# eBay/Sequence-Semantic-Embedding

Measured on AMD Instinct MI355X. Metric: encoded seqs/sec (+ query x target cosine-scores/sec, top-1 vs ref), higher is better.
Workload: dtype f32; 1 GPU; configs[1]: classification stand-in, dual-encoder LSTM H=S=256 E=50 T=32 V=32000; encode 16384 source seqs/GPU/step + cosine top-10 vs 571-target index; batch_per_gpu=16384, seq_len=32, targets=571, parallelism=dp1, weights=random-init (reference initialisers, seed 0)

## Files before the change

### sequence-semantic-embedding_amd/csrc/score_topk.hip

```cpp
#include <cstdlib>

#include "sse_kernels.h"
#include "score_exact.h"

#define SC_THREADS 512
#define SC_KC 16
#ifndef SC_PRIO_K
#define SC_PRIO_K 1
#define SC_PRIO_E 0
#endif

#ifdef SSE_SCORE_CLOCK
#include <cstdio>
__device__ long long g_score_clk[8 * 8];
#define SC_CLK_DECL long long ck_[8] = {0, 0, 0, 0, 0, 0, 0, 0}, ck_t = clock64();
#define SC_CLK(i)                   \
  {                                 \
    const long long n_ = clock64(); \
    ck_[i] += n_ - ck_t;            \
    ck_t = n_;                      \
  }
#else
#define SC_CLK_DECL
#define SC_CLK(i)
// ... 983 lines not shown
      col[row] = (row < a.N) ? acc[r] : NEG_INF;
    }
  }
  SC_CLK(1)
  __syncthreads();
  SC_CLK(2)
  if (NT * 32 <= 640) {
    si_select4<10>(a, sc, NP, NT, qt, w * 8, lane SI_CLK_ARGS);
    SC_CLK(3)
    si_select4<10>(a, sc, NP, NT, qt, w * 8 + 4, lane SI_CLK_ARGS);
    SC_CLK(4)
#ifdef SSE_SCORE_CLOCK
    if (blockIdx.x == gridDim.x / 2 && lane == 0)
      for (int i = 0; i < 8; ++i) g_score_clk[w * 8 + i] = ck_[i];
#endif
  } else {
    si_select4<16>(a, sc, NP, NT, qt, w * 8, lane SI_CLK_ARGS);
    si_select4<16>(a, sc, NP, NT, qt, w * 8 + 4, lane SI_CLK_ARGS);
  }
}
template <int KB>
__global__ __launch_bounds__(256) void score_small_index_x3_kernel(SmallIndexArgs a) {
  extern __shared__ __attribute__((aligned(16))) float si_sc[];
  const int tid = threadIdx.x, lane = tid & 63, w = __builtin_amdgcn_readfirstlane(tid >> 6);
  const int NT = a.NT, NP = NT * 32 + 1;
  const int qt = blockIdx.x;
  float *sc = si_sc;
  SC_CLK_DECL
  sse_u32x4 bh[KB], bl[KB];
  {
    const int row = qt * 32 + (lane & 31), kb0 = (lane >> 5) * 8;
    const float *src = a.q_rows + (size_t)(row < a.Q ? row : 0) * a.S + kb0;
    const bool vec = (a.S & 3) == 0 && (reinterpret_cast<uintptr_t>(a.q_rows) & 15) == 0 && KB * 16 <= a.S;
#pragma unroll
    for (int kb = 0; kb < KB; ++kb) {
      float v[8] = {0, 0, 0, 0, 0, 0, 0, 0};
      if (vec) {
        const f32x4 v0 = *reinterpret_cast<const f32x4 *>(src + kb * 16), v1 = *reinterpret_cast<const f32x4 *>(src + kb * 16 + 4);
#pragma unroll
        for (int e = 0; e < 4; ++e) {
          v[e] = v0[e];
          v[4 + e] = v1[e];
        }
      } else {
#pragma unroll
        for (int e = 0; e < 8; ++e)
          if (kb * 16 + kb0 + e < a.S) v[e] = src[kb * 16 + e];
      }
      if (row >= a.Q) {
#pragma unroll
        for (int e = 0; e < 8; ++e) v[e] = 0.0f;
      }
      sse_split8(v, bh[kb], bl[kb]);
    }
  }
  SC_CLK(0)
  {
    constexpr int D = KB < 4 ? KB : 4;
    static_assert(KB % D == 0, "the ring index must be static");
    const sse_u32x4 *img = reinterpret_cast<const sse_u32x4 *>(a.idx_x3) + lane;
    const sse_u32x4 *ap = img + (size_t)(w < NT ? w : 0) * KB * 128;
    sse_u32x4 ah[D], al[D];
#pragma unroll
    for (int d = 0; d < D; ++d) {
      ah[d] = ap[d * 128];
      al[d] = ap[d * 128 + 64];
    }
    for (int t = w; t < NT; t += 4) {
      const sse_u32x4 *apn = img + (size_t)(t + 4 < NT ? t + 4 : t) * KB * 128;
      f32x16 acc = {0, 0, 0, 0, 0, 0, 0, 0, 0, 0, 0, 0, 0, 0, 0, 0};
#pragma unroll
      for (int kb = 0; kb < KB; ++kb) {
        __builtin_amdgcn_sched_barrier(0);
        const bf16x8_t xh = __builtin_bit_cast(bf16x8_t, ah[kb % D]), xl = __builtin_bit_cast(bf16x8_t, al[kb % D]);
        const bf16x8_t yh = __builtin_bit_cast(bf16x8_t, bh[kb]), yl = __builtin_bit_cast(bf16x8_t, bl[kb]);
        acc = __builtin_amdgcn_mfma_f32_32x32x16_bf16(xh, yh, acc, 0, 0, 0);
        acc = __builtin_amdgcn_mfma_f32_32x32x16_bf16(xh, yl, acc, 0, 0, 0);
        acc = __builtin_amdgcn_mfma_f32_32x32x16_bf16(xl, yh, acc, 0, 0, 0);
        __builtin_amdgcn_sched_barrier(0);
        const sse_u32x4 *nx = (kb + D < KB) ? ap + (kb + D) * 128 : apn + (kb + D - KB) * 128;
        ah[kb % D] = nx[0];
        al[kb % D] = nx[64];
      }
      const int rb = t * 32 + 4 * (lane >> 5);
      float *col = sc + (lane & 31) * NP;
#pragma unroll
      for (int r = 0; r < 16; ++r) {
        const int row = rb + (r & 3) + 8 * (r >> 2);
        col[row] = (row < a.N) ? acc[r] : NEG_INF;
      }
      ap = apn;
    }
  }
  SC_CLK(1)
  __syncthreads();
  SC_CLK(2)
  if (NT * 32 <= 640) {
    si_select4<10>(a, sc, NP, NT, qt, w * 8, lane SI_CLK_ARGS);
    SC_CLK(3)
    si_select4<10>(a, sc, NP, NT, qt, w * 8 + 4, lane SI_CLK_ARGS);
    SC_CLK(4)
#ifdef SSE_SCORE_CLOCK
    if (blockIdx.x == gridDim.x / 2 && lane == 0)
      for (int i = 0; i < 8; ++i) g_score_clk[w * 8 + i] = ck_[i];
#endif
  } else {
    si_select4<16>(a, sc, NP, NT, qt, w * 8, lane SI_CLK_ARGS);
    si_select4<16>(a, sc, NP, NT, qt, w * 8 + 4, lane SI_CLK_ARGS);
  }
}
bool score_small_index_applies(int Q, int KG, int64_t NT) {
  return Q >= 1024 && (KG == 32 || KG == 8 || KG == 7) && NT * 32 <= 1024 && (size_t)32 * (NT * 32 + 1) * sizeof(float) <= (size_t)144 * 1024;
}
hipError_t launch_score_small_index(const SmallIndexArgs &a, hipStream_t stream) {
  if (!score_small_index_applies(a.Q, a.KG, a.NT)) return hipErrorInvalidValue;
  const size_t lds = (size_t)32 * (a.NT * 32 + 1) * sizeof(float);
  const dim3 grid((a.Q + 31) / 32), block(256);
  auto go = [&](auto kernel) -> hipError_t {
    hipError_t e = hipFuncSetAttribute(reinterpret_cast<const void *>(kernel), hipFuncAttributeMaxDynamicSharedMemorySize, (int)lds);
    if (e != hipSuccess) return e;
    hipLaunchKernelGGL(kernel, grid, block, lds, stream, a);
    return hipGetLastError();
  };
  if (a.idx_x3 && a.KG != 32) return go(score_small_index_x3_kernel<4>);
  if (a.KG == 8) return go(score_small_index_kernel<8>);
  if (a.KG == 7) return go(score_small_index_kernel<7>);
  const hipError_t e32 = a.idx_x3 ? go(score_small_index_x3_kernel<16>) : go(score_small_index_kernel<32>);
  if (e32 != hipSuccess) return e32;
#ifdef SSE_SCORE_CLOCK
  if (a.Q >= 8192) {
    static int n = 0;
    if (n++ % 8 == 3) {
      long long v[64];
      (void)hipStreamSynchronize(stream);
      (void)hipMemcpyFromSymbol(v, HIP_SYMBOL(g_score_clk), sizeof v);
      for (int w = 0; w < 4; w += 3)
        fprintf(stderr, "[small index clock Q=%d NT=%d] wave %d cycles: query fragments %lld | scores (MFMA + LDS stores) %lld | barrier %lld | selection: loads + bounds %lld | bisection %lld | winners + rank + stores %lld (both batches)\n",
                a.Q, a.NT, w, v[w * 8 + 0], v[w * 8 + 1], v[w * 8 + 2], v[w * 8 + 5], v[w * 8 + 6], v[w * 8 + 3] + v[w * 8 + 4]);
    }
  }
#endif
  return hipGetLastError();
}

hipError_t launch_score_topk(const ScoreArgs &a_in, hipStream_t stream) {
  ScoreArgs a = a_in;
#ifdef SSE_SCORE_MEASURE
  {
    static const int dbg = getenv("SSE_SCORE_DBG") ? atoi(getenv("SSE_SCORE_DBG")) : 0;
// ... 11 lines not shown
    if (a.NQ == 2) return launch_score_variant<2, false, true>(a, stream);
    if (a.NQ == 4) return launch_score_variant<4, false, true>(a, stream);
    return hipErrorInvalidValue;
  }
  if (!a.part_bnd) return hipErrorInvalidValue;
  if (a.BF) {
    if (a.NQ == 1) return launch_score_variant<1, true, false>(a, stream);
    if (a.NQ == 2) return launch_score_variant<2, true, false>(a, stream);
    if (a.NQ == 4) return launch_score_variant<4, true, false>(a, stream);
    return hipErrorInvalidValue;
  }
  if (a.NQ == 1) return launch_score_variant<1, false, false>(a, stream);
  if (a.NQ == 2) return launch_score_variant<2, false, false>(a, stream);
  if (a.NQ == 4) return launch_score_variant<4, false, false>(a, stream);
  return hipErrorInvalidValue;
}


template <int NB>
__device__ __forceinline__ int packed_value_of_lane(int lane) {
  int v = 0;
#pragma unroll
  for (int cnt = NB, bit = 5; cnt > 1; cnt >>= 1, --bit) v = v * 2 + ((lane >> bit) & 1);
  return v;
}
template <int NB>
__device__ __forceinline__ int packed_lane_of_value(int v) {
  int lane = 0;
#pragma unroll
  for (int cnt = NB, bit = 5; cnt > 1; cnt >>= 1, --bit) lane |= ((v / (cnt / 2)) & 1) << bit;
  return lane;
}
template <int NB>
__device__ __forceinline__ double wave_exact_dot_packed(const float *qrow, const float *idxp, const double *idx64, const int64_t (&n)[NB],
                                                        int S, int KG, int lane, const float *idx_rm = nullptr) {
  static_assert(NB == 2 || NB == 4 || NB == 8, "power of two");
  double acc[NB];
#pragma unroll
  for (int b = 0; b < NB; ++b) acc[b] = 0.0;
  if (idx64) {
    for (int d = lane; d < S; d += 64) {
      double rv[NB];
#pragma unroll
      for (int b = 0; b < NB; ++b) rv[b] = idx64[(size_t)n[b] * S + d];
#pragma unroll
      for (int b = 0; b < NB; ++b) acc[b] += (double)qrow[d] * rv[b];
    }
  } else {
    for (int j = lane; j < KG * 2; j += 64) {
      const int kg = j >> 1, half = j & 1;
      f32x4 v[NB];
#pragma unroll
      for (int b = 0; b < NB; ++b)
        v[b] = idx_rm ? *reinterpret_cast<const f32x4 *>(idx_rm + (size_t)n[b] * S + j * 4)
                      : *reinterpret_cast<const f32x4 *>(idxp + (size_t)(n[b] >> 5) * KG * 256 + kg * 256 + (half * 32 + (int)(n[b] & 31)) * 4);
      const int d0 = kg * 8 + half * 4;
#pragma unroll
      for (int e = 0; e < 4; ++e)
        if (d0 + e < S) {
#pragma unroll
          for (int b = 0; b < NB; ++b) acc[b] += (double)qrow[d0 + e] * (double)v[b][e];
        }
    }
  }
  int m = 32;
#pragma unroll
  for (int cnt = NB; cnt > 1; cnt >>= 1, m >>= 1) {
    const bool up = (lane & m) != 0;
#pragma unroll
    for (int i = 0; i < cnt / 2; ++i) {
      const double send = up ? acc[i] : acc[i + cnt / 2];
      const double keep = up ? acc[i + cnt / 2] : acc[i];
      acc[i] = keep + __shfl_xor(send, m);
    }
  }
#pragma unroll
  for (; m > 0; m >>= 1) acc[0] += __shfl_xor(acc[0], m);
  return acc[0];
}

#define RS_THREADS 256
#define RS_MAXWIN 256
#define RS_MAXNC 4096
__global__ __launch_bounds__(RS_THREADS) void rescore_kernel(RescoreArgs a) {
  __shared__ int s_cnt;
  __shared__ int s_wid[RS_MAXWIN];
  __shared__ double s_ex[RS_MAXWIN];
  __shared__ float s_m[RS_THREADS / 64];
  __shared__ double s_qn[RS_THREADS / 64];
  extern __shared__ __attribute__((aligned(16))) unsigned long long s_key[];
  const int q = blockIdx.x, tid = threadIdx.x, lane = tid & 63, w = tid >> 6;
  if (a.uncert_clear && q == 0 && tid == 0) *a.uncert_clear = 0;
  if (a.q_count && q >= *a.q_count) return;
  const int qo = a.qmap ? a.qmap[q] : q;
  const float *ps = a.part_scores + (size_t)q * a.NC;
  const int32_t *pi = a.part_ids + (size_t)q * a.NC;
  const float *qrow = a.q + (size_t)q * a.S;
  const int KG = (a.S + 7) / 8;

  constexpr int PER = RS_MAXNC / RS_THREADS;
  float rs[PER];
  int ri[PER];
#pragma unroll
  for (int j = 0; j < PER; ++j) {
    const int c = tid + j * RS_THREADS;
    ri[j] = (c < a.NC) ? pi[c] : -1;
    rs[j] = (c < a.NC) ? ps[c] : NEG_INF;
  }
  float mmax = NEG_INF;
  for (int c = tid; c < a.NC / SC_KC; c += RS_THREADS) mmax = fmaxf(mmax, a.part_bnd[(size_t)q * (a.NC / SC_KC) + c]);

// ... 225 lines not shown
    a.out_ids[(size_t)qo * a.k + r2] = a.id_base + idm;
    if (a.host_flag) {
      a.host_scores[(size_t)qo * a.k + r2] = exm;
      a.host_ids[(size_t)qo * a.k + r2] = a.id_base + idm;
    }
  }
  const unsigned long long tmask = __ballot(member && r2 == a.k - 1);
  const double theta = tmask ? readlane_f64(exm, __ffsll((long long)tmask) - 1) : -__builtin_inf();
  if (a.host_flag) __threadfence_system();
  RS_CLK(3)
#ifdef SSE_SCORE_CLOCK
  if (q == a.Q / 2 && lane == 0) {
    rk_[4] = nwin;
    for (int i = 0; i < 6; ++i) g_score_clk[i] = rk_[i];
  }
#endif
  if (lane == 0) {
    const bool ok = (nwin >= a.k) && ((double)mmax + (double)eps_q < theta);
    a.cert[qo] = ok ? 1 : 0;
    if (!ok && a.uncert) atomicAdd(a.uncert, 1);
    if (a.col_thr) a.col_thr[qo] = ok ? __builtin_inff() : __double2float_rd(theta - (double)(a.eps32 * qnorm));
    if (a.col_slot) {
      a.col_slot[qo] = ok ? -1 : qo;
      a.col_cnt[qo] = 0;
    }
    if (a.host_flag) {
      a.host_cert[qo] = ok ? 1 : 0;
      if (qo == 0 && a.host_err) *a.host_err = a.err_in ? *a.err_in : 0;
      __hip_atomic_store(a.host_flag + qo, a.seq, __ATOMIC_RELEASE, __HIP_MEMORY_SCOPE_SYSTEM);
    }
  }
}

hipError_t launch_rescore(const RescoreArgs &a, hipStream_t stream) {
  if (a.NC > RS_MAXNC) return hipErrorInvalidValue;
  if (a.NC <= 64) {
    hipLaunchKernelGGL(rescore_small_kernel, dim3((a.Q + 3) / 4), dim3(256), 0, stream, a);
#ifdef SSE_SCORE_CLOCK
    if (a.Q >= 8192) {
      static int n = 0;
      if (n++ % 8 == 3) {
        long long v[8];
        (void)hipStreamSynchronize(stream);
        (void)hipMemcpyFromSymbol(v, HIP_SYMBOL(g_score_clk), sizeof v);
        fprintf(stderr, "[rescore_small clock Q=%d NC=%d] cycles: query norm %lld | candidates, rank, k-th, window %lld | float64 dots %lld (window of %lld) | exact rank + outputs %lld\n",
                a.Q, a.NC, v[0], v[1], v[2], v[4], v[3]);
      }
    }
#endif
    return hipGetLastError();
  }
  hipLaunchKernelGGL(rescore_kernel, dim3(a.Q), dim3(RS_THREADS), (size_t)a.NC * sizeof(unsigned long long), stream, a);
  return hipGetLastError();
}

#define EX_THREADS 256
struct ExactArgs {
  const float *q;
  const float *idxp;
  const double *idx64;
  const int32_t *cert;
  double *out_scores;
  int64_t *out_ids;
  int64_t id_base, N;
  int32_t Q, S, k;
  int32_t k_off, k_total;
  unsigned long long *served;
  const int32_t *uncert;
};

__device__ __forceinline__ void exact_topk_query(const ExactArgs a, const int q, double (*s_sc)[SC_KC],
                                                 int64_t (*s_id)[SC_KC]) {
  const int tid = threadIdx.x, lane = tid & 63, w = tid >> 6;
  if (a.served && tid == 0 && a.k_off == 0) atomicAdd(a.served, 1ull);
  const float *qrow = a.q + (size_t)q * a.S;
  const int KG = (a.S + 7) / 8;
  double ls[SC_KC];
// ... 177 lines not shown
  for (int o = 32; o > 0; o >>= 1) qn += __shfl_xor(qn, o);
  float v[4];
#pragma unroll
  for (int j = 0; j < 4; ++j) v[j] = (j * 64 + lane < NV) ? lane_max[(size_t)qi * NV + j * 64 + lane] : -__builtin_inff();
  float kth = -__builtin_inff();
  for (int round = 0; round < 16; ++round) {
    float m = fmaxf(fmaxf(v[0], v[1]), fmaxf(v[2], v[3]));
#pragma unroll
    for (int o = 32; o > 0; o >>= 1) m = fmaxf(m, __shfl_xor(m, o));
    kth = m;
    const unsigned long long has = __ballot(v[0] == m || v[1] == m || v[2] == m || v[3] == m);
    if (has == 0ull) break;
    if (lane == __ffsll((long long)has) - 1) {
      if (v[0] == m) v[0] = -__builtin_inff();
      else if (v[1] == m) v[1] = -__builtin_inff();
      else if (v[2] == m) v[2] = -__builtin_inff();
      else v[3] = -__builtin_inff();
    }
  }
  if (lane == 0) {
    float thr = -__builtin_inff();
    if (kth > -__builtin_inff() && kth == kth) thr = __double2float_rd((double)kth - 2.0 * (double)eps * sqrt(qn));
    col_thr[qi] = thr;
    col_slot[qi] = qi;
  }
}
hipError_t launch_lane_max_threshold(const float *q, const float *lane_max, int Q, int S, int NV, float eps, float *col_thr,
                                     int32_t *col_slot, hipStream_t st) {
  if (NV < 16 || NV > 256) return hipErrorInvalidValue;
  hipLaunchKernelGGL(lane_max_threshold_kernel, dim3((Q + 3) / 4), dim3(256), 0, st, q, lane_max, Q, S, NV, eps, col_thr, col_slot);
  return hipGetLastError();
}

__device__ __forceinline__ void select_topk_query(const SelectArgs &a, const int q, unsigned long long *sel_smem) {
  const int tid = threadIdx.x, lane = tid & 63, w = tid >> 6;
  const int slot = a.col_slot[q];
  if (slot < 0) return;
  const int n = a.col_cnt[slot];
  if (n > a.col_cap || n < a.k) return;
  int n2 = 1;
  while (n2 < n) n2 <<= 1;
  unsigned long long *skey = sel_smem;
  int *srow = reinterpret_cast<int *>(sel_smem + n2);
  const int32_t *rows = a.col_buf + (size_t)slot * a.col_cap;
  const float *qrow = a.q + (size_t)q * a.S;
  const int KG = (a.S + 7) / 8;
  for (int i = w; i < n2; i += 4) {
    if (i < n) {
      const int row = rows[i];
      const double ex = wave_exact_dot(qrow, a.idx32, a.idx64, row, a.S, KG, lane);
      if (lane == 0) {
        unsigned long long u = (unsigned long long)__double_as_longlong(ex);
        u = (u >> 63) ? ~u : (u | 0x8000000000000000ull);
        skey[i] = u;
        srow[i] = row;
      }
    } else if (lane == 0) {
      skey[i] = 0ull;
      srow[i] = 0x7FFFFFFF;
    }
  }
  for (int size = 2; size <= n2; size <<= 1)
    for (int stride = size >> 1; stride > 0; stride >>= 1) {
      __syncthreads();
      for (int i = tid; i < (n2 >> 1); i += 256) {
        const int lo = 2 * i - (i & (stride - 1)), hi = lo + stride;
        const bool desc = ((lo & size) == 0);
        const unsigned long long x = skey[lo], y = skey[hi];
        const int rx = srow[lo], ry = srow[hi];
        const bool x_after_y = (x < y) || (x == y && rx > ry);
        if (x_after_y == desc) {
          skey[lo] = y;
          skey[hi] = x;
          srow[lo] = ry;
          srow[hi] = rx;
        }
      }
    }
  __syncthreads();
  for (int j = tid; j < a.k; j += 256) {
    unsigned long long u = skey[j];
    u = (u >> 63) ? (u & 0x7FFFFFFFFFFFFFFFull) : ~u;
    a.out_scores[(size_t)q * a.k + j] = __longlong_as_double((long long)u);
    a.out_ids[(size_t)q * a.k + j] = a.id_base + srow[j];
  }
  if (tid == 0) {
    a.cert[q] = 1;
    if (a.served) atomicAdd(a.served, 1ull);
  }
}
__global__ __launch_bounds__(256) void select_topk_kernel(SelectArgs a) {
  extern __shared__ __attribute__((aligned(16))) unsigned long long sel_smem[];
  __shared__ unsigned char s_open[256];
  if (a.uncert && *a.uncert == 0) return;
  {
    const long long q = (long long)blockIdx.x + (long long)threadIdx.x * gridDim.x;
    s_open[threadIdx.x] = (q < a.Q) && a.col_slot[q] >= 0;
  }
  __syncthreads();
  int it = 0;
#pragma nounroll
  for (int q = blockIdx.x; q < a.Q; q += gridDim.x, ++it) {
    const bool open = it < 256 ? s_open[it] != 0 : a.col_slot[q] >= 0;
    if (!open) continue;
    select_topk_query(a, q, sel_smem);
    __syncthreads();
  }
}
hipError_t launch_select_topk(const SelectArgs &a, hipStream_t st) {
  if (a.col_cap > SSE_COLLECT_CAP) return hipErrorInvalidValue;
  const size_t lds = (size_t)a.col_cap * (sizeof(unsigned long long) + sizeof(int));
  hipError_t e = hipFuncSetAttribute(reinterpret_cast<const void *>(select_topk_kernel), hipFuncAttributeMaxDynamicSharedMemorySize, (int)lds);
  if (e != hipSuccess) return e;
  const int grid = (a.uncert && a.grid_cap > 0 && a.grid_cap < a.Q) ? a.grid_cap : a.Q;
  hipLaunchKernelGGL(select_topk_kernel, dim3(grid), dim3(256), lds, st, a);
  return hipGetLastError();
}

__global__ void merge_topk_kernel(const double *in_s, const int64_t *in_i, int64_t stride, int P, int Q, int k, double *out_s,
                                  int64_t *out_i) {
  const int q = blockIdx.x * blockDim.x + threadIdx.x;
  if (q >= Q) return;
  for (int p = 0; p < P; ++p)
    for (int j = 0; j < k; ++j) {
      const double s = in_s[(size_t)p * stride + (size_t)q * k + j];
      const int64_t id = in_i[(size_t)p * stride + (size_t)q * k + j];
      int rank = j;
      for (int p2 = 0; p2 < P && rank < k; ++p2) {
        if (p2 == p) continue;
        for (int j2 = 0; j2 < k; ++j2) {
          const double s2 = in_s[(size_t)p2 * stride + (size_t)q * k + j2];
          const int64_t id2 = in_i[(size_t)p2 * stride + (size_t)q * k + j2];
          if (before(s2, id2, s, id)) ++rank; else break;
        }
      }
      if (rank < k) {
        out_s[(size_t)q * k + rank] = s;
        out_i[(size_t)q * k + rank] = id;
      }
    }
}

hipError_t launch_merge_topk(const double *in_s, const int64_t *in_i, int64_t stride, int P, int Q, int k, double *out_s,
                             int64_t *out_i, hipStream_t stream) {
  hipLaunchKernelGGL(merge_topk_kernel, dim3((Q + 127) / 128), dim3(128), 0, stream, in_s, in_i, stride, P, Q, k, out_s,
                     out_i);
  return hipGetLastError();
}
// ... 1 lines not shown
```

### sequence-semantic-embedding_amd/csrc/sse_api.hip

```cpp
#include <cmath>
#include <cstdarg>
#include <cstdio>
#include <cstdlib>
#include <algorithm>
#include <chrono>
#include <cstring>
#include <dlfcn.h>
#include <link.h>
#include <mutex>
#include <string>
#include <vector>

#include "../../include/sse_hip.h"
#include "sse_kernels.h"
#include "train.h"

namespace {

thread_local std::string g_create_error;

struct Variable {
  std::string name;
  int rows = 0, cols = 0;
  int64_t count = 0;
// ... 88 lines not shown
  bool pad_skip = true;
  int pad_sort_dev = 1;
  int64_t score_two_pass_min_rows = 49152, score_two_pass_rows = 524288;
  int64_t two_pass_calls = 0;
  DevBuf s_lmax;
  bool lstm_gate_split = true;
  DevBuf s_padzero, s_padwork, s_padorder;
  int32_t *pad_stat = nullptr;
  int32_t pad_seq = 0;
  int64_t pad_sorted_calls = 0;
  int64_t lstm_path_calls[10] = {0, 0, 0, 0, 0, 0, 0, 0, 0, 0};
  bool lstm_x3 = false;
  unsigned short *emb16 = nullptr;
  bool emb16_valid = false;
  int lstm_persist_rows = 32;
  uint32_t persist_epoch = 0;
  hipStream_t stream = nullptr;
  bool persist_inject = false;
  int64_t persist_fallbacks = 0;
  int cu_count = 0;
  int lstm_cluster_rows = 1024;
  uint32_t cluster_epoch = 0;
  int lstm_cluster_chunks = 3;
  int cluster_backoff = -1;
  int cluster_skip[2] = {0, 0};
  int lstm_cluster_coop = 1;
  int lstm_cluster_wt = 0;
  int lstm_cluster_drop = 0;
  int lstm_small_rows = 1024;
  int lstm_x_table = 1;
  int lstm_x_table_mb = 256;
  int64_t x_table_builds = 0;
  bool score_small_index = true;
  bool score_small_x3 = true;
  bool score_bf16 = true;
  void *idxp16 = nullptr;
  size_t idxp16_cap = 0;
  bool idxp16_valid = false;
  bool fb_cnt_init = false;
  int uncert_word = 0;
  bool cnn_bf16 = false;
  unsigned short *emb_bf16 = nullptr, *cnn_Wc16 = nullptr, *cnn_Mx3 = nullptr;
  int lstm_train_rows = 0;
  bool train_bwd_x3 = false;
  bool train_fwd_x3 = false;
  bool train_dk_x3 = false;
  bool train_generic = false;
  bool train_gen1 = false;
  bool train_pair_dedup = true;
  bool train_serial = false;
  float *emb_pad = nullptr;
  int cnn_W[4] = {-1, -1, -1, -1}, cnn_b[4] = {-1, -1, -1, -1}, cnn_M = -1, tgt_table = -1;
  float *cnn_Wc = nullptr, *cnn_bias = nullptr, *cnn_Mp = nullptr;
  int32_t *err_flag = nullptr;
  float *idxp = nullptr;
  size_t idxp_cap = 0;
  double *idx64 = nullptr;
  DevBuf idx_rm;
  bool idx_rm_valid = false;
  DevBuf idx_x3;
  bool idx_x3_valid = false;
  int64_t idx_N = 0, idx_base = 0;
  int idx_S = 0;
  float idx_norm_max = 1.0f;
  DevBuf s_ids, s_out, s_q, s_qp, s_ps, s_pi, s_cert, s_os, s_oi, s_tmp, s_tmp2, s_feat, s_zero, s_map;
  DevBuf s_qmap, s_qc;
// ... 1206 lines not shown
  r.q = q;
  r.idx32 = h->idxp;
  r.idx64 = h->idx64;
  r.idx_rm = h->idx_rm_valid ? (const float *)h->idx_rm.p : nullptr;
  r.part_scores = a.part_scores;
  r.part_ids = a.part_ids;
  r.part_bnd = a.part_bnd;
  r.out_scores = out_s;
  r.out_ids = out_i;
  r.cert = (int32_t *)h->s_cert.p;
  r.id_base = h->idx_base;
  r.N = h->idx_N;
  r.Q = Q;
  r.S = S;
  r.NC = NC;
  r.k = k;
  const float eps32 = (float)(2.0 * (S + 2) * 5.97e-8 * h->idx_norm_max);
  r.eps = eps32;
  r.eps32 = eps32;
  r.col_thr = (float *)h->s_cthr.p;
  if (first) h->uncert_word ^= 1;
  int32_t *const uncert = (int32_t *)(counters + 4) + h->uncert_word;
  const int follow_grid = 2 * (h->cu_count > 0 ? h->cu_count : 256);
  r.uncert = uncert;
  r.uncert_clear = (int32_t *)(counters + 4) + (h->uncert_word ^ 1);
  const bool own_slots = Q <= POOL;
  if (own_slots) {
    r.col_slot = (int32_t *)h->s_cslot.p;
    r.col_cnt = (int32_t *)h->s_ccnt.p;
  }
  if (bf) r.eps += (float)(1.02 * (1.0 / 256.0 + 1.0 / 262144.0) * h->idx_norm_max);
  if (small_x3)
    r.eps = (float)(((1.0 + 1.0 / 64.0) / 32768.0 + 2.0 * (3 * S + 2) * 5.97e-8 * (1.0 + 1.0 / 32.0)) * h->idx_norm_max);
  if (first) {
    RescoreArgs rf = r;
    if (mirror) {
      rf.host_scores = mirror->scores;
      rf.host_ids = mirror->ids;
      rf.host_cert = mirror->cert;
      rf.host_err = mirror->err;
      rf.host_flag = mirror->flag;
      rf.err_in = h->err_flag;
      rf.seq = mirror->seq;
    }
    HIPCHECK(h, launch_rescore(rf, st));
  }
  if (!rest) return 0;
  const float *qp32 = (const float *)h->s_qp.p;
  if (bf && Q > 32) {
    if (reserve(h, h->s_qp32, (size_t)QB * NQ * KG * 256 * sizeof(float))) return 1;
    if (reserve(h, h->s_qmap, (size_t)(Q + 1) * sizeof(int32_t))) return 1;
    if (reserve(h, h->s_qc, (size_t)QT * 32 * S * sizeof(float))) return 1;
    HIPCHECK(h, launch_count_uncert(r.cert, Q, counters, st));
    int32_t *qmap = (int32_t *)h->s_qmap.p, *qcount = qmap + Q;
    HIPCHECK(h, launch_compact_uncert(q, r.cert, Q, S, qmap, qcount, (float *)h->s_qc.p, st));
    if (!rows_direct) HIPCHECK(h, launch_pack_rows((const float *)h->s_qc.p, Q, S, (float *)h->s_qp32.p, st));
    ScoreArgs a2 = a;
    a2.BF = 0;
    a2.idxp = h->idxp;
    a2.qp = (const float *)h->s_qp32.p;
    if (rows_direct) a2.q_rows = (const float *)h->s_qc.p;
    a2.KG = KG;
    a2.q_count = qcount;
    a2.NSPLIT = nsplit2;
    HIPCHECK(h, launch_score_topk(a2, st));
    RescoreArgs r2 = r;
    r2.q = (const float *)h->s_qc.p;
    r2.NC = nsplit2 * 16;
    r2.eps = eps32;
    r2.qmap = qmap;
    r2.q_count = qcount;
    r2.uncert = r2.uncert_clear = nullptr;
    HIPCHECK(h, launch_rescore(r2, st));
    qp32 = (const float *)h->s_qp32.p;
  }
  if (!own_slots) {
    HIPCHECK(h, hipMemsetAsync(h->s_ccnt.p, 0, (size_t)(POOL + 1) * sizeof(int32_t), st));
    HIPCHECK(h, launch_assign_slots(r.cert, Q, POOL, (int32_t *)h->s_cslot.p, (int32_t *)h->s_ccnt.p + POOL, st));
  }
  ScoreArgs c = a;
  c.BF = 0;
  c.idxp = h->idxp;
  c.qp = qp32;
  c.q_rows = q;
  c.S = S;
  c.KG = KG;
  c.COLLECT = 1;
  c.col_thr = (const float *)h->s_cthr.p;
  c.col_slot = (const int32_t *)h->s_cslot.p;
  c.col_cnt = (int32_t *)h->s_ccnt.p;
  c.col_buf = (int32_t *)h->s_cbuf.p;
  c.col_cap = SSE_COLLECT_CAP;
  c.uncert = uncert;
  HIPCHECK(h, launch_score_topk(c, st));
  SelectArgs sel{q, h->idxp, h->idx64, c.col_slot, c.col_cnt, c.col_buf, SSE_COLLECT_CAP, out_s, out_i, r.cert, h->idx_base, Q, S, k,
                 counters + 1, uncert, follow_grid};
  HIPCHECK(h, launch_select_topk(sel, st));
  HIPCHECK(h, launch_exact_topk(q, h->idxp, h->idx64, r.cert, out_s, out_i, h->idx_base, h->idx_N, Q, S, k, st, counters + 2, uncert,
                                follow_grid));
  return 0;
}

}

extern "C" {

const char *sse_last_error(sse_handle *h) { return h ? h->err.c_str() : g_create_error.c_str(); }

int sse_create(const sse_config *cfg, sse_handle **out) {
  if (!cfg || !out) return fail(nullptr, "sse_create: null argument");
  *out = nullptr;
  int ndev = 0;
  if (hipGetDeviceCount(&ndev) != hipSuccess || ndev == 0) return fail(nullptr, "no HIP device available");
  if (cfg->device < 0 || cfg->device >= ndev) return fail(nullptr, "device %d out of range (have %d)", cfg->device, ndev);
  if (cfg->vocab_size < 2 || cfg->embedding_size < 1 || cfg->encoding_size < 1)
    return fail(nullptr, "bad model sizes V=%d E=%d S=%d", cfg->vocab_size, cfg->embedding_size, cfg->encoding_size);
  sse_handle *h = new sse_handle();
  h->cfg = *cfg;
  h->lr = cfg->learning_rate;
#define CREATE_FAIL(...)        \
  do {                          \
    fail(nullptr, __VA_ARGS__); \
    sse_destroy(h);             \
    return 1;                   \
  } while (0)
  if (hipSetDevice(cfg->device) != hipSuccess) CREATE_FAIL("hipSetDevice(%d) failed", cfg->device);
  add_var(h, "word_embedding", cfg->vocab_size, cfg->embedding_size);
  switch (cfg->network_mode) {
    case SSE_MODE_DUAL_ENCODER:
      setup_encoder(h, h->enc[0], "source_encoder", "source_encoder/src_M", cfg->src_cell_size, cfg->src_cell_size);
      setup_encoder(h, h->enc[1], "target_encoder", "target_encoder/tgt_M", cfg->tgt_cell_size, cfg->tgt_cell_size);
      break;
// ... 396 lines not shown
  }
  static const char *const above_names[3] = {"score_above_band_rows", "score_above_bruteforce_pairs", "score_above_long_segments"};
  for (int i = 0; i < 3; ++i) {
    if (strcmp(name, above_names[i]) != 0) continue;
    unsigned long long v[3] = {0, 0, 0};
    if (h->s_ab_cnt.p && h->ab_cnt_init) {
      HIPCHECK(h, hipSetDevice(h->cfg.device));
      HIPCHECK(h, hipDeviceSynchronize());
      HIPCHECK(h, hipMemcpy(v, h->s_ab_cnt.p, sizeof v, hipMemcpyDeviceToHost));
    }
    *value = (int64_t)v[i];
    return 0;
  }
  static const char *const names[3] = {"score_bf16_second_chance_queries", "score_collect_queries", "score_bruteforce_queries"};
  for (int i = 0; i < 3; ++i) {
    if (strcmp(name, names[i]) != 0) continue;
    unsigned long long v[4] = {0, 0, 0, 0};
    if (h->s_fb_cnt.p && h->fb_cnt_init) {
      HIPCHECK(h, hipSetDevice(h->cfg.device));
      HIPCHECK(h, hipDeviceSynchronize());
      HIPCHECK(h, hipMemcpy(v, h->s_fb_cnt.p, sizeof v, hipMemcpyDeviceToHost));
    }
    *value = (int64_t)v[i];
    return 0;
  }
  return fail(h, "unknown counter '%s'", name);
}

int sse_set_option(sse_handle *h, const char *name, int32_t value) {
  if (!h || !name) return 1;
  std::lock_guard<std::mutex> lk(h->mu);
  if (strcmp(name, "score_small_index") == 0) {
    h->score_small_index = value != 0;
    return 0;
  }
  if (strcmp(name, "score_small_x3") == 0) {
    h->score_small_x3 = value != 0;
    return 0;
  }
  if (strcmp(name, "score_bf16") == 0) {
    h->score_bf16 = value != 0;
    return 0;
  }
  if (strcmp(name, "cnn_bf16") == 0) {
    if (h->cfg.network_mode != SSE_MODE_SOURCE_ONLY_CNN) return fail(h, "option cnn_bf16 needs network_mode source_only_cnn");
    h->cnn_bf16 = value != 0;
    h->packed_dirty = true;
    h->mp_fresh = false;
    return 0;
  }
  if (strcmp(name, "lstm_train_rows") == 0) {
    if (value != 0 && value != 32 && value != 64) return fail(h, "lstm_train_rows must be 0, 32 or 64");
    h->lstm_train_rows = (int)value;
    return 0;
  }
  if (strcmp(name, "train_bwd_x3") == 0) {
    h->train_bwd_x3 = value != 0;
    return 0;
  }
  if (strcmp(name, "train_fwd_x3") == 0) {
    h->train_fwd_x3 = value != 0;
    return 0;
  }
  if (strcmp(name, "train_dk_x3") == 0) {
    h->train_dk_x3 = value != 0;
    return 0;
// ... 1343 lines not shown
```

### sequence-semantic-embedding_amd/csrc/sse_kernels.h

```cpp
#pragma once
#include <hip/hip_runtime.h>
#include <stdint.h>

typedef float f32x4 __attribute__((ext_vector_type(4)));
typedef float f32x16 __attribute__((ext_vector_type(16)));

__host__ __device__ static inline int frag32_off(int r_in_tile, int k_in_group) {
  return ((((k_in_group >> 2) << 5) + r_in_tile) << 2) + (k_in_group & 3);
}

__device__ static inline int mfma_row(int reg, int lane) { return (reg & 3) + 8 * (reg >> 2) + 4 * (lane >> 5); }

static inline int round_up(int x, int m) { return (x + m - 1) / m * m; }

typedef unsigned int sse_u32x4 __attribute__((ext_vector_type(4)));
__host__ __device__ static inline unsigned short sse_bf16_rne(float f) {
  unsigned u;
  __builtin_memcpy(&u, &f, 4);
  u += 0x7FFFu + ((u >> 16) & 1u);
  return (unsigned short)(u >> 16);
}
__host__ __device__ static inline float sse_bf16_f32(unsigned short h) {
  const unsigned u = (unsigned)h << 16;
  float f;
// ... 225 lines not shown
hipError_t launch_count_uncert(const int32_t *cert, int Q, unsigned long long *count, hipStream_t st);
hipError_t launch_compact_uncert(const float *q, const int32_t *cert, int Q, int S, int32_t *qmap, int32_t *count, float *qc,
                                 hipStream_t st);
hipError_t launch_frag32_to_bf16(const float *idxp, int64_t NT, int KG, void *out, hipStream_t stream);
hipError_t launch_frag32_to_split_bf16(const float *idxp, int64_t NT, int KG, void *out, hipStream_t stream);

#define SSE_COLLECT_CAP 4096
#define SSE_MAX_SELECT_K 1024

struct RescoreArgs {
  const float *q;
  const float *idx32;
  const double *idx64;
  const float *part_scores;
  const int32_t *part_ids;
  const float *part_bnd;
  double *out_scores;
  int64_t *out_ids;
  int32_t *cert;
  int64_t id_base, N;
  int32_t Q, S, NC, k;
  float eps;
  const int32_t *qmap = nullptr, *q_count = nullptr;
  float *col_thr = nullptr;
  float eps32 = 0.0f;
  int32_t *col_slot = nullptr, *col_cnt = nullptr;
  double *host_scores = nullptr;
  int64_t *host_ids = nullptr;
  int32_t *host_cert = nullptr, *host_flag = nullptr, *host_err = nullptr;
  const int32_t *err_in = nullptr;
  int32_t seq = 0;
  const float *idx_rm = nullptr;
  int32_t *uncert = nullptr, *uncert_clear = nullptr;
};
hipError_t launch_rescore(const RescoreArgs &a, hipStream_t stream);

struct SmallIndexArgs {
  const float *q_rows;
  const float *idxp;
  float *part_scores;
  int32_t *part_ids;
  float *part_bnd;
  int64_t N;
  int32_t Q, S, KG, NT;
  const void *idx_x3 = nullptr;
};
bool score_small_index_applies(int Q, int KG, int64_t NT);
hipError_t launch_score_small_index(const SmallIndexArgs &a, hipStream_t stream);

struct RankArgs {
  const float *q;
  const int32_t *pair_q;
  const int64_t *pair_id;
  const double *pair_score_in;
  const float *idxp;
  const double *idx64;
  int64_t *out_before;
  double *out_score;
  double *thr64;
  float *lo, *hi;
  unsigned long long *sure;
  int32_t *band_cnt, *band_buf;
  int32_t band_cap;
  const int32_t *bad;
  unsigned long long *counters;
  int64_t id_base, N;
// ... 40 lines not shown
  const int64_t *offsets;
  const unsigned long long *cursor;
  int64_t *ids;
  double *scores;
  int64_t *scratch_ids;
  double *scratch_scores;
  const int32_t *bad;
  int32_t *err_flag;
  unsigned long long *counters;
  int64_t L, cap, id_base, N;
  int32_t S, KG;
};
hipError_t launch_above_lists(const AboveListArgs &a, hipStream_t st);

hipError_t launch_assign_slots(const int32_t *cert, int Q, int slots, int32_t *col_slot, int32_t *counter, hipStream_t st);
hipError_t launch_kth_bound(const float *q, const float *part_scores, const int32_t *part_ids, int Q, int S, int NC, int k,
                            float eps, float *col_thr, int32_t *col_slot, hipStream_t st);
struct SelectArgs {
  const float *q;
  const float *idx32;
  const double *idx64;
  const int32_t *col_slot, *col_cnt, *col_buf;
  int32_t col_cap;
  double *out_scores;
  int64_t *out_ids;
  int32_t *cert;
  int64_t id_base;
  int32_t Q, S, k;
  unsigned long long *served = nullptr;
  const int32_t *uncert = nullptr;
  int32_t grid_cap = 0;
};
hipError_t launch_select_topk(const SelectArgs &a, hipStream_t st);

hipError_t launch_merge_topk(const double *in_s, const int64_t *in_i, int64_t stride, int P, int Q, int k, double *out_s,
                             int64_t *out_i, hipStream_t stream);

hipError_t launch_pack_rows(const float *rows, int64_t R, int C, float *out, hipStream_t stream);
hipError_t launch_pack_rows_norm(const float *rows, int64_t R, int C, float *out, float *norm_bits, hipStream_t stream);
hipError_t launch_f64_to_f32(const double *in, float *out, int64_t n, hipStream_t stream);
hipError_t launch_l2_normalize(const float *x, float *out, int64_t rows, int cols, hipStream_t stream);

hipError_t launch_pack_lstm(const float *K, const float *b, int E, int H, int Ep, int Hp, int UB, float *Wp,
                            hipStream_t stream);
enum { PACK_JOB_PAD_ROWS = 1, PACK_JOB_LSTM = 2, PACK_JOB_KN = 3, PACK_JOB_KT = 4 };
struct PackJob {
  int32_t type;
  const float *a, *b;
  float *out;
  int64_t total;
  int32_t i0, i1, i2, i3;
};
#define SSE_MAX_PACK_JOBS 12
struct PackJobs {
  PackJob job[SSE_MAX_PACK_JOBS];
  int32_t n = 0;
};
void pack_job_pad_rows(PackJobs &js, const float *in, int64_t R, int C, int Cp, int one_col, float *out);
void pack_job_lstm(PackJobs &js, const float *K, const float *b, int E, int H, int Ep, int Hp, float *Wp);
void pack_job_kn(PackJobs &js, const float *X, int K, int N, int KGp, float *out);
void pack_job_kT(PackJobs &js, const float *K, int row0, int nrows, int RT, int H, int Hp, float *out);
hipError_t launch_pack_multi(const PackJobs &js, hipStream_t stream);
hipError_t launch_pack_kn(const float *X, int K, int N, int KGp, float *out, hipStream_t stream);
hipError_t launch_pad_rows(const float *in, int64_t R, int C, int Cp, int one_col, float *out, hipStream_t stream);
#define SSE_PAD_SORT_MAX_T 8192
size_t pad_sort_zeroed_words();
// ... 29 lines not shown
```

Before: 7.625 million seqs/s.

## Add four-query-per-wave rescore, stage query loads via LDS, fuse follow-up kernels

Adds a rescore kernel that handles four queries per wave with 16 lanes each. It uses DPP rotations for in-group ranking and can use the already-sorted candidate list from the small-index path. The small-index x3 scoring kernel now loads query rows cooperatively into LDS with coalesced vector loads before splitting them into registers. The select-topk and exact-topk fallback launches are merged into one follow-up kernel that exits early when nothing is uncertain. Together these cut launch count and wave underuse in the scoring tail, at the cost of more code paths and an extra LDS staging pass with barriers.

Measured after the change: 7.676 million seqs/s (median of 6 runs). No clear change (+0.7%).

```diff
diff --git a/sequence-semantic-embedding_amd/csrc/score_topk.hip b/sequence-semantic-embedding_amd/csrc/score_topk.hip
--- a/sequence-semantic-embedding_amd/csrc/score_topk.hip
+++ b/sequence-semantic-embedding_amd/csrc/score_topk.hip
@@ -1039,26 +1039,43 @@
     const int row = qt * 32 + (lane & 31), kb0 = (lane >> 5) * 8;
     const float *src = a.q_rows + (size_t)(row < a.Q ? row : 0) * a.S + kb0;
     const bool vec = (a.S & 3) == 0 && (reinterpret_cast<uintptr_t>(a.q_rows) & 15) == 0 && KB * 16 <= a.S;
-#pragma unroll
-    for (int kb = 0; kb < KB; ++kb) {
-      float v[8] = {0, 0, 0, 0, 0, 0, 0, 0};
-      if (vec) {
-        const f32x4 v0 = *reinterpret_cast<const f32x4 *>(src + kb * 16), v1 = *reinterpret_cast<const f32x4 *>(src + kb * 16 + 4);
+    if (vec) {
+      constexpr int SP = KB * 16 + 4, RV = KB * 4;
+      const f32x4 *g4 = reinterpret_cast<const f32x4 *>(a.q_rows + (size_t)qt * 32 * a.S);
+      const int rows_in = min(32, a.Q - qt * 32);
+#pragma unroll
+      for (int i0 = 0; i0 < 32 * RV; i0 += 256) {
+        const int i = i0 + tid, r = i / RV, c = i - r * RV;
+        const f32x4 v = (r < rows_in) ? g4[i] : f32x4{0, 0, 0, 0};
+        *reinterpret_cast<f32x4 *>(sc + r * SP + c * 4) = v;
+      }
+      __syncthreads();
+      const float *ls = sc + (lane & 31) * SP + kb0;
+#pragma unroll
+      for (int kb = 0; kb < KB; ++kb) {
+        const f32x4 v0 = *reinterpret_cast<const f32x4 *>(ls + kb * 16), v1 = *reinterpret_cast<const f32x4 *>(ls + kb * 16 + 4);
+        float v[8];
 #pragma unroll
         for (int e = 0; e < 4; ++e) {
           v[e] = v0[e];
           v[4 + e] = v1[e];
         }
-      } else {
+        sse_split8(v, bh[kb], bl[kb]);
+      }
+      __syncthreads();
+    } else {
+#pragma unroll
+      for (int kb = 0; kb < KB; ++kb) {
+        float v[8] = {0, 0, 0, 0, 0, 0, 0, 0};
 #pragma unroll
         for (int e = 0; e < 8; ++e)
           if (kb * 16 + kb0 + e < a.S) v[e] = src[kb * 16 + e];
-      }
-      if (row >= a.Q) {
-#pragma unroll
-        for (int e = 0; e < 8; ++e) v[e] = 0.0f;
-      }
-      sse_split8(v, bh[kb], bl[kb]);
+        if (row >= a.Q) {
+#pragma unroll
+          for (int e = 0; e < 8; ++e) v[e] = 0.0f;
+        }
+        sse_split8(v, bh[kb], bl[kb]);
+      }
     }
   }
   SC_CLK(0)
@@ -1121,7 +1138,11 @@
 }
 hipError_t launch_score_small_index(const SmallIndexArgs &a, hipStream_t stream) {
   if (!score_small_index_applies(a.Q, a.KG, a.NT)) return hipErrorInvalidValue;
-  const size_t lds = (size_t)32 * (a.NT * 32 + 1) * sizeof(float);
+  size_t lds = (size_t)32 * (a.NT * 32 + 1) * sizeof(float);
+  if (a.idx_x3) {
+    const size_t stage = (size_t)32 * ((a.KG == 32 ? 16 : 4) * 16 + 4) * sizeof(float);
+    lds = lds > stage ? lds : stage;
+  }
   const dim3 grid((a.Q + 31) / 32), block(256);
   auto go = [&](auto kernel) -> hipError_t {
     hipError_t e = hipFuncSetAttribute(reinterpret_cast<const void *>(kernel), hipFuncAttributeMaxDynamicSharedMemorySize, (int)lds);
@@ -1199,6 +1220,23 @@
   return lane;
 }
 template <int NB>
+__device__ __forceinline__ double packed_reduce(double (&acc)[NB], int lane) {
+  int m = 32;
+#pragma unroll
+  for (int cnt = NB; cnt > 1; cnt >>= 1, m >>= 1) {
+    const bool up = (lane & m) != 0;
+#pragma unroll
+    for (int i = 0; i < cnt / 2; ++i) {
+      const double send = up ? acc[i] : acc[i + cnt / 2];
+      const double keep = up ? acc[i + cnt / 2] : acc[i];
+      acc[i] = keep + __shfl_xor(send, m);
+    }
+  }
+#pragma unroll
+  for (; m > 0; m >>= 1) acc[0] += __shfl_xor(acc[0], m);
+  return acc[0];
+}
+template <int NB>
 __device__ __forceinline__ double wave_exact_dot_packed(const float *qrow, const float *idxp, const double *idx64, const int64_t (&n)[NB],
                                                         int S, int KG, int lane, const float *idx_rm = nullptr) {
   static_assert(NB == 2 || NB == 4 || NB == 8, "power of two");
@@ -1230,20 +1268,7 @@
         }
     }
   }
-  int m = 32;
-#pragma unroll
-  for (int cnt = NB; cnt > 1; cnt >>= 1, m >>= 1) {
-    const bool up = (lane & m) != 0;
-#pragma unroll
-    for (int i = 0; i < cnt / 2; ++i) {
-      const double send = up ? acc[i] : acc[i + cnt / 2];
-      const double keep = up ? acc[i + cnt / 2] : acc[i];
-      acc[i] = keep + __shfl_xor(send, m);
-    }
-  }
-#pragma unroll
-  for (; m > 0; m >>= 1) acc[0] += __shfl_xor(acc[0], m);
-  return acc[0];
+  return packed_reduce<NB>(acc, lane);
 }
 
 #define RS_THREADS 256
@@ -1535,10 +1560,145 @@
   }
 }
 
+#define RQ_ROR15(STEP) STEP(1) STEP(2) STEP(3) STEP(4) STEP(5) STEP(6) STEP(7) STEP(8) STEP(9) STEP(10) STEP(11) STEP(12) STEP(13) STEP(14) STEP(15)
+#define RQ_ROR(x, n) __builtin_amdgcn_update_dpp((x), (x), 0x120 + (n), 0xF, 0xF, false)
+__global__ __launch_bounds__(256) void rescore_quad_kernel(RescoreArgs a) {
+  const int lane = threadIdx.x & 63, g = lane >> 4, s = lane & 15, row0 = lane & 48;
+  const int wave = __builtin_amdgcn_readfirstlane((int)(threadIdx.x >> 6));
+  const int q0 = (blockIdx.x * 4 + wave) * 4;
+  if (a.uncert_clear && blockIdx.x == 0 && threadIdx.x == 0) *a.uncert_clear = 0;
+  const int Qeff = a.q_count ? min(a.Q, *a.q_count) : a.Q;
+  if (q0 >= Qeff) return;
+  const int nq = min(4, Qeff - q0);
+  const bool valid = g < nq;
+  const int q = q0 + (valid ? g : nq - 1);
+  const int qo = a.qmap ? a.qmap[q] : q;
+  const int KG = (a.S + 7) / 8;
+#ifdef SSE_SCORE_CLOCK
+  long long rk_[6] = {0, 0, 0, 0, 0, 0}, rk_t = clock64();
+#endif
+  const int id = a.part_ids[(size_t)q * SC_KC + s];
+  const float sc = a.part_scores[(size_t)q * SC_KC + s];
+  const float bnd = a.part_bnd[q];
+  double qn;
+  {
+    double acc[4] = {0.0, 0.0, 0.0, 0.0};
+    const float *qr[4];
+#pragma unroll
+    for (int c = 0; c < 4; ++c) qr[c] = a.q + (size_t)(q0 + min(c, nq - 1)) * a.S;
+    for (int d = lane; d < a.S; d += 64) {
+#pragma unroll
+      for (int c = 0; c < 4; ++c) acc[c] += (double)qr[c][d] * qr[c][d];
+    }
+    qn = packed_reduce<4>(acc, lane);
+  }
+  const float qnorm = (float)sqrt(qn);
+  const float eps_q = a.eps * qnorm;
+  RS_CLK(0)
+
+  float kth;
+  if (a.sorted) {
+    const int ks = a.k - 1;
+    const float ksc = __shfl(sc, row0 | (ks & 15));
+    const int kid = __shfl(id, row0 | (ks & 15));
+    kth = (ks < SC_KC && kid >= 0) ? ksc : NEG_INF;
+  } else {
+    unsigned u = __float_as_uint(sc);
+    u = (u & 0x80000000u) ? ~u : (u | 0x80000000u);
+    const unsigned long long key = (id < 0) ? 0ull : (((unsigned long long)u << 32) | (unsigned long long)(0xFFFFFFFFu - (unsigned)id));
+    const int key_lo = (int)(unsigned)key, key_hi = (int)(unsigned)(key >> 32);
+    int rank = 0;
+#define RQ_STEP(n)                                                                                                            \
+  {                                                                                                                           \
+    const unsigned long long kj = ((unsigned long long)(unsigned)RQ_ROR(key_hi, n) << 32) | (unsigned long long)(unsigned)RQ_ROR(key_lo, n); \
+    rank += (kj > key) ? 1 : 0;                                                                                               \
+  }
+    RQ_ROR15(RQ_STEP)
+#undef RQ_STEP
+    const unsigned long long kmask = __ballot(key != 0ull && rank == a.k - 1);
+    const unsigned kg = (unsigned)(kmask >> row0) & 0xFFFFu;
+    const float ksc = __shfl(sc, row0 | (kg ? __ffs((int)kg) - 1 : 0));
+    kth = kg ? ksc : NEG_INF;
+  }
+  const bool in_win = valid && (id >= 0) && (sc >= kth - 2.0f * eps_q);
+  const float mmax = fmaxf(NEG_INF, bnd);
+  const unsigned long long wmask = __ballot(in_win);
+  const unsigned wg = (unsigned)(wmask >> row0) & 0xFFFFu;
+  const int nwin = __popc(wg);
+  const int mi = __popc(wg & ((1u << s) - 1u));
+  const int idm = __builtin_amdgcn_ds_permute((row0 | (in_win ? mi : 15)) * 4, id);
+  RS_CLK(1)
+  double exm = -__builtin_inf();
+  for (int c = 0; c < nq; ++c) {
+    const int nw = __popc((unsigned)(wmask >> (16 * c)) & 0xFFFFu);
+    const float *qrow = a.q + (size_t)(q0 + c) * a.S;
+    for (int m0 = 0; m0 < nw; m0 += RS_NB) {
+      int64_t n[RS_NB];
+#pragma unroll
+      for (int i = 0; i < RS_NB; ++i) n[i] = __builtin_amdgcn_readlane(idm, 16 * c + ((m0 + i < nw) ? m0 + i : 0));
+      const double tot = wave_exact_dot_packed<RS_NB>(qrow, a.idx32, a.idx64, n, a.S, KG, lane, a.idx_rm);
+      const int want = s - m0;
+      const double got = __shfl(tot, packed_lane_of_value<RS_NB>(want & (RS_NB - 1)));
+      if (g == c && want >= 0 && want < RS_NB && s < nw) exm = got;
+    }
+  }
+  RS_CLK(2)
+  const bool member = s < nwin;
+  int r2 = 0;
+  {
+    const long long eb = __double_as_longlong(member ? exm : -__builtin_inf());
+    const int e_lo = (int)eb, e_hi = (int)(eb >> 32), e_id = member ? idm : 0x7FFFFFFF;
+#define RQ_STEP(n)                                                                                                         \
+  {                                                                                                                        \
+    const double os = __longlong_as_double(((long long)RQ_ROR(e_hi, n) << 32) | (long long)(unsigned)RQ_ROR(e_lo, n));      \
+    r2 += before(os, (int64_t)RQ_ROR(e_id, n), exm, (int64_t)idm) ? 1 : 0;                                                  \
+  }
+    RQ_ROR15(RQ_STEP)
+#undef RQ_STEP
+  }
+  if (member && r2 < a.k) {
+    a.out_scores[(size_t)qo * a.k + r2] = exm;
+    a.out_ids[(size_t)qo * a.k + r2] = a.id_base + idm;
+    if (a.host_flag) {
+      a.host_scores[(size_t)qo * a.k + r2] = exm;
+      a.host_ids[(size_t)qo * a.k + r2] = a.id_base + idm;
+    }
+  }
+  const unsigned long long tmask = __ballot(member && r2 == a.k - 1);
+  const unsigned tg = (unsigned)(tmask >> row0) & 0xFFFFu;
+  const double tsc = __shfl(exm, row0 | (tg ? __ffs((int)tg) - 1 : 0));
+  const double theta = tg ? tsc : -__builtin_inf();
+  if (a.host_flag) __threadfence_system();
+  RS_CLK(3)
+#ifdef SSE_SCORE_CLOCK
+  if (q0 <= a.Q / 2 && a.Q / 2 < q0 + 4 && lane == 0) {
+    rk_[4] = __popcll(wmask);
+    for (int i = 0; i < 6; ++i) g_score_clk[i] = rk_[i];
+  }
+#endif
+  if (s == 0 && valid) {
+    const bool ok = (nwin >= a.k) && ((double)mmax + (double)eps_q < theta);
+    a.cert[qo] = ok ? 1 : 0;
+    if (!ok && a.uncert) atomicAdd(a.uncert, 1);
+    if (a.col_thr) a.col_thr[qo] = ok ? __builtin_inff() : __double2float_rd(theta - (double)(a.eps32 * qnorm));
+    if (a.col_slot) {
+      a.col_slot[qo] = ok ? -1 : qo;
+      a.col_cnt[qo] = 0;
+    }
+    if (a.host_flag) {
+      a.host_cert[qo] = ok ? 1 : 0;
+      if (qo == 0 && a.host_err) *a.host_err = a.err_in ? *a.err_in : 0;
+      __hip_atomic_store(a.host_flag + qo, a.seq, __ATOMIC_RELEASE, __HIP_MEMORY_SCOPE_SYSTEM);
+    }
+  }
+}
+
 hipError_t launch_rescore(const RescoreArgs &a, hipStream_t stream) {
   if (a.NC > RS_MAXNC) return hipErrorInvalidValue;
   if (a.NC <= 64) {
-    hipLaunchKernelGGL(rescore_small_kernel, dim3((a.Q + 3) / 4), dim3(256), 0, stream, a);
+    const bool quad = a.NC == SC_KC && a.quad;
+    if (quad) hipLaunchKernelGGL(rescore_quad_kernel, dim3((a.Q + 15) / 16), dim3(256), 0, stream, a);
+    else hipLaunchKernelGGL(rescore_small_kernel, dim3((a.Q + 3) / 4), dim3(256), 0, stream, a);
 #ifdef SSE_SCORE_CLOCK
     if (a.Q >= 8192) {
       static int n = 0;
@@ -1546,6 +1706,7 @@
         long long v[8];
         (void)hipStreamSynchronize(stream);
         (void)hipMemcpyFromSymbol(v, HIP_SYMBOL(g_score_clk), sizeof v);
+        if (quad) fprintf(stderr, "[rescore_quad clock: one wave = 4 queries, window = the four windows together]\n");
         fprintf(stderr, "[rescore_small clock Q=%d NC=%d] cycles: query norm %lld | candidates, rank, k-th, window %lld | float64 dots %lld (window of %lld) | exact rank + outputs %lld\n",
                 a.Q, a.NC, v[0], v[1], v[2], v[4], v[3]);
       }
@@ -1789,12 +1950,12 @@
   return hipGetLastError();
 }
 
-__device__ __forceinline__ void select_topk_query(const SelectArgs &a, const int q, unsigned long long *sel_smem) {
+__device__ __forceinline__ bool select_topk_query(const SelectArgs &a, const int q, unsigned long long *sel_smem) {
   const int tid = threadIdx.x, lane = tid & 63, w = tid >> 6;
   const int slot = a.col_slot[q];
-  if (slot < 0) return;
+  if (slot < 0) return false;
   const int n = a.col_cnt[slot];
-  if (n > a.col_cap || n < a.k) return;
+  if (n > a.col_cap || n < a.k) return false;
   int n2 = 1;
   while (n2 < n) n2 <<= 1;
   unsigned long long *skey = sel_smem;
@@ -1845,6 +2006,7 @@
     a.cert[q] = 1;
     if (a.served) atomicAdd(a.served, 1ull);
   }
+  return true;
 }
 __global__ __launch_bounds__(256) void select_topk_kernel(SelectArgs a) {
   extern __shared__ __attribute__((aligned(16))) unsigned long long sel_smem[];
@@ -1871,6 +2033,41 @@
   if (e != hipSuccess) return e;
   const int grid = (a.uncert && a.grid_cap > 0 && a.grid_cap < a.Q) ? a.grid_cap : a.Q;
   hipLaunchKernelGGL(select_topk_kernel, dim3(grid), dim3(256), lds, st, a);
+  return hipGetLastError();
+}
+
+__global__ __launch_bounds__(EX_THREADS) void follow_up_kernel(SelectArgs a, ExactArgs x) {
+  extern __shared__ __attribute__((aligned(16))) unsigned long long sel_smem[];
+  __shared__ unsigned char s_open[EX_THREADS];
+  if (a.uncert && *a.uncert == 0) return;
+  auto flags = [&](long long q) -> int { return (q < a.Q) ? (a.col_slot[q] >= 0 ? 1 : 0) | (a.cert[q] == 0 ? 2 : 0) : 0; };
+  s_open[threadIdx.x] = (unsigned char)flags((long long)blockIdx.x + (long long)threadIdx.x * gridDim.x);
+  __syncthreads();
+  double(*s_sc)[SC_KC] = reinterpret_cast<double(*)[SC_KC]>(sel_smem);
+  int64_t(*s_id)[SC_KC] = reinterpret_cast<int64_t(*)[SC_KC]>(sel_smem + (EX_THREADS / 64) * SC_KC);
+  int it = 0;
+#pragma nounroll
+  for (int q = blockIdx.x; q < a.Q; q += gridDim.x, ++it) {
+    const int open = it < EX_THREADS ? s_open[it] : flags(q);
+    if (!open) continue;
+    const bool served = (open & 1) && select_topk_query(a, q, sel_smem);
+    __syncthreads();
+    if ((open & 2) && !served) {
+      exact_topk_query(x, q, s_sc, s_id);
+      __syncthreads();
+    }
+  }
+}
+hipError_t launch_follow_up(const SelectArgs &a, int64_t N, unsigned long long *bf_served, hipStream_t st) {
+  if (a.col_cap > SSE_COLLECT_CAP || a.k > SC_KC || !a.uncert || !a.cert) return hipErrorInvalidValue;
+  const size_t lists = (size_t)(EX_THREADS / 64) * SC_KC * (sizeof(double) + sizeof(int64_t));
+  const size_t sort = (size_t)a.col_cap * (sizeof(unsigned long long) + sizeof(int));
+  const size_t lds = sort > lists ? sort : lists;
+  hipError_t e = hipFuncSetAttribute(reinterpret_cast<const void *>(follow_up_kernel), hipFuncAttributeMaxDynamicSharedMemorySize, (int)lds);
+  if (e != hipSuccess) return e;
+  const ExactArgs x{a.q, a.idx32, a.idx64, a.cert, a.out_scores, a.out_ids, a.id_base, N, a.Q, a.S, a.k, 0, a.k, bf_served, a.uncert};
+  const int grid = (a.grid_cap > 0 && a.grid_cap < a.Q) ? a.grid_cap : a.Q;
+  hipLaunchKernelGGL(follow_up_kernel, dim3(grid), dim3(EX_THREADS), lds, st, a, x);
   return hipGetLastError();
 }
 
diff --git a/sequence-semantic-embedding_amd/csrc/sse_api.hip b/sequence-semantic-embedding_amd/csrc/sse_api.hip
--- a/sequence-semantic-embedding_amd/csrc/sse_api.hip
+++ b/sequence-semantic-embedding_amd/csrc/sse_api.hip
@@ -144,6 +144,7 @@
   int lstm_x_table_mb = 256;
   int64_t x_table_builds = 0;
   bool score_small_index = true;
+  bool score_rescore_quad = true;
   bool score_small_x3 = true;
   bool score_bf16 = true;
   void *idxp16 = nullptr;
@@ -1416,8 +1417,10 @@
   if (bf) r.eps += (float)(1.02 * (1.0 / 256.0 + 1.0 / 262144.0) * h->idx_norm_max);
   if (small_x3)
     r.eps = (float)(((1.0 + 1.0 / 64.0) / 32768.0 + 2.0 * (3 * S + 2) * 5.97e-8 * (1.0 + 1.0 / 32.0)) * h->idx_norm_max);
+  r.quad = h->score_rescore_quad ? 1 : 0;
   if (first) {
     RescoreArgs rf = r;
+    rf.sorted = small_idx ? 1 : 0;
     if (mirror) {
       rf.host_scores = mirror->scores;
       rf.host_ids = mirror->ids;
@@ -1479,9 +1482,7 @@
   HIPCHECK(h, launch_score_topk(c, st));
   SelectArgs sel{q, h->idxp, h->idx64, c.col_slot, c.col_cnt, c.col_buf, SSE_COLLECT_CAP, out_s, out_i, r.cert, h->idx_base, Q, S, k,
                  counters + 1, uncert, follow_grid};
-  HIPCHECK(h, launch_select_topk(sel, st));
-  HIPCHECK(h, launch_exact_topk(q, h->idxp, h->idx64, r.cert, out_s, out_i, h->idx_base, h->idx_N, Q, S, k, st, counters + 2, uncert,
-                                follow_grid));
+  HIPCHECK(h, launch_follow_up(sel, h->idx_N, counters + 2, st));
   return 0;
 }
 
@@ -1944,6 +1945,10 @@
   std::lock_guard<std::mutex> lk(h->mu);
   if (strcmp(name, "score_small_index") == 0) {
     h->score_small_index = value != 0;
+    return 0;
+  }
+  if (strcmp(name, "score_rescore_quad") == 0) {
+    h->score_rescore_quad = value != 0;
     return 0;
   }
   if (strcmp(name, "score_small_x3") == 0) {
diff --git a/sequence-semantic-embedding_amd/csrc/sse_kernels.h b/sequence-semantic-embedding_amd/csrc/sse_kernels.h
--- a/sequence-semantic-embedding_amd/csrc/sse_kernels.h
+++ b/sequence-semantic-embedding_amd/csrc/sse_kernels.h
@@ -281,6 +281,7 @@
   int32_t seq = 0;
   const float *idx_rm = nullptr;
   int32_t *uncert = nullptr, *uncert_clear = nullptr;
+  int32_t quad = 0, sorted = 0;
 };
 hipError_t launch_rescore(const RescoreArgs &a, hipStream_t stream);
 
@@ -387,6 +388,7 @@
   int32_t grid_cap = 0;
 };
 hipError_t launch_select_topk(const SelectArgs &a, hipStream_t st);
+hipError_t launch_follow_up(const SelectArgs &a, int64_t N, unsigned long long *bf_served, hipStream_t st);
 
 hipError_t launch_merge_topk(const double *in_s, const int64_t *in_i, int64_t stride, int P, int Q, int k, double *out_s,
                              int64_t *out_i, hipStream_t stream);
```
